# ZhengyiLuo/PULSE

Hardware: AMD Instinct MI355X
Metric: env-steps/sec through PPO update (higher is better)
Workload: dtype f32; 1 GPU; cfg2: 4096 SMPL-humanoid envs/GPU x horizon 32, imitation obs/reward/reset + PPO (actor+critic MLP [1024, 512], minibatch 16384 x 6 mini-epochs); num_envs_per_gpu=4096, horizon=32, global_batch=131072, parallelism=dp1, reference_motion=HBM-resident motion library (1024 clips), queried every step

## Files before the change

### include/pulse_hip.h

```cpp
#ifndef PULSE_HIP_H
#define PULSE_HIP_H

#include <stddef.h>
#include <stdint.h>

#ifdef __cplusplus
extern "C" {
#endif

#define PULSE_OK 0
#define PULSE_ERR_INVALID_ARG (-1)
#define PULSE_ERR_LAUNCH (-2)
#define PULSE_ERR_UNSUPPORTED (-3)

#define PULSE_ABI_VERSION 34

typedef void* pulse_stream_t;

int pulse_abi_version(void);
const char* pulse_last_error(void);

int pulse_quat_mul(const float* a, const float* b, float* out, int64_t m, pulse_stream_t s);
int pulse_quat_conjugate(const float* a, float* out, int64_t m, pulse_stream_t s);
int pulse_quat_rotate(const float* q, const float* v, float* out, int64_t m, pulse_stream_t s);
int pulse_quat_to_angle_axis(const float* q, float* angle, float* axis, int64_t m, pulse_stream_t s);
int pulse_quat_to_exp_map(const float* q, float* out, int64_t m, pulse_stream_t s);
int pulse_quat_to_tan_norm(const float* q, float* out, int64_t m, pulse_stream_t s);
int pulse_exp_map_to_quat(const float* e, float* out, int64_t m, pulse_stream_t s);
int pulse_slerp(const float* q0, const float* q1, const float* t, float* out, int64_t m, pulse_stream_t s);
int pulse_calc_heading(const float* q, float* out, int64_t m, pulse_stream_t s);
int pulse_calc_heading_quat(const float* q, float* out, int64_t m, int inverse, pulse_stream_t s);

typedef struct pulse_motion_tables {
    const float* frames;
    int64_t frame_stride;
    int64_t total_frames;
    int32_t num_bodies;
    int32_t off_gts, off_grs, off_lrs, off_gvs, off_gavs, off_dvs;
    const float* motion_lengths;
    const float* motion_dt;
    const int64_t* motion_num_frames;
    const int64_t* length_starts;
    int32_t num_motions;
} pulse_motion_tables;

typedef struct pulse_reward_specs {
    float k_pos, k_rot, k_vel, k_ang_vel;
    float w_pos, w_rot, w_vel, w_ang_vel;
    float power_coef;
    int32_t power_reward;
} pulse_reward_specs;

#define PULSE_IM_SELF_OBS 1u
#define PULSE_IM_TASK_OBS 2u
#define PULSE_IM_REWARD   4u
#define PULSE_IM_RESET    8u
#define PULSE_IM_DEBUG_POISON_LDS 0x80000000u
#define PULSE_IM_FORCE_WIDE 0x40000000u

typedef struct pulse_im_step_args {
    const float* rb;
    int64_t rb_env_stride;
    int32_t num_envs;
    int32_t num_bodies;
    const int64_t* env_ids;
    int32_t num_ids;
    const uint8_t* env_mask;

// ... 178 lines not shown
    const int64_t* clip_out_start;
    const int64_t* clip_frames_host;
    const float* clip_dt;
    const float* clip_heading;
    const float* local_translation;
    const int32_t* parent_indices_host;
    float* frames;
    int64_t total_frames;
    int64_t frame_stride;
    int32_t off_gts, off_grs, off_lrs, off_gvs, off_gavs, off_dvs;
    float filter_w[9];
} pulse_motion_build_args;
int pulse_sizeof_motion_build_args(void);
int pulse_motion_build(const pulse_motion_build_args* args, pulse_stream_t s);

typedef struct pulse_im_eval_args {
    const float* rb;
    int64_t rb_env_stride;
    const float* ref_pos;
    int64_t ref_env_stride;
    int32_t num_envs;
    int32_t num_bodies;
    const int32_t* num_steps;
    int32_t step;
    const uint8_t* env_mask;
    float* ring;
    double* accum;
    int64_t accum_stride;
} pulse_im_eval_args;
int pulse_sizeof_im_eval_args(void);
int pulse_im_eval_accum(const pulse_im_eval_args* args, pulse_stream_t s);

typedef struct pulse_rollout_record_args {
    int32_t num_envs;
    const float* rewards;
    float reward_scale, reward_shift;
    const int64_t* dones;
    const int64_t* terminate;
    const float* value_raw; int64_t value_stride;
    const double* value_mean; const double* value_var;
    float value_eps;
    float* buf_rewards; float* buf_next_values; uint8_t* buf_dones; int64_t env_stride;
    float* current_rewards; float* current_lengths;
    float* meter_rewards; float* meter_lengths;
    float meter_max_size;
    uint8_t* done_mask;
    uint8_t* buf_terminate;
    float* meter_partials; int32_t meter_blocks;
} pulse_rollout_record_args;
int pulse_sizeof_rollout_record_args(void);
int pulse_rollout_record(const pulse_rollout_record_args* args, pulse_stream_t s);
int pulse_rollout_meters(const float* partials, int32_t steps, int32_t blocks, float* meter_rewards, float* meter_lengths, float meter_max_size,
                         pulse_stream_t s);

int pulse_kinematic_sim_step(const float* target_rb, const float* noise_rb, float* rb, int64_t num_envs, int32_t num_bodies,
                             const float* target_dof_pos, const float* noise_dof_pos, float* dof_pos,
                             const float* target_dof_vel, const float* noise_dof_vel, float* dof_vel,
                             const float* force_src, float* dof_force, int32_t num_dof, pulse_stream_t s);

typedef struct pulse_pd_sim_args {
    int64_t num_envs; int32_t num_bodies;
    const float* target_rb;
    const float* target_dof_pos; const float* target_dof_vel;
    const float* action;
    const float* noise_acc;
    const float* sag;
    const float* lever_dir;
    float kp, kd, dt, action_scale, lever; int32_t substeps;
    float* err; float* err_vel;
    float* rb; float* dof_pos; float* dof_vel; float* dof_force;
    const uint8_t* reset_mask;
} pulse_pd_sim_args;
int pulse_sizeof_pd_sim_args(void);
int pulse_pd_sim_step(const pulse_pd_sim_args* args, pulse_stream_t s);

typedef struct pulse_traj_step_args {
    uint32_t what; int32_t num_envs;
    const int64_t* env_ids; int32_t num_ids; const uint8_t* env_mask;
    const float* rb; int64_t rb_env_stride; int32_t num_bodies;
    int32_t upright_start;
    const int64_t* progress; float dt;
    const float* verts; int32_t num_verts; float traj_dur;
    int32_t num_samples; float sample_timestep;
    const int16_t* heightsamples; int32_t map_rows, map_cols; float horizontal_scale, vertical_scale;
    const float* height_points; int32_t num_height_points; int32_t sensor_body;
    const float* center_points; int32_t num_center_points; int32_t use_center_height; float height_meas_scale;
    const float* dof_force; const float* dof_vel; int32_t num_dof; float power_coef; int32_t power_reward; int32_t fuzzy_target;
    const float* contact_forces; const int32_t* contact_body_ids; int32_t num_contact_ids; const float* termination_heights;
    float max_episode_length, fail_dist; int32_t enable_early_termination, terrain_reset, disable_collision;
    float* obs; int64_t obs_stride; int32_t obs_offset;
    float* rew; float* rew_raw;
    int64_t* reset; int64_t* terminate;
} pulse_traj_step_args;
int pulse_sizeof_traj_step_args(void);
int pulse_traj_step(const pulse_traj_step_args* args, pulse_stream_t s);

typedef struct pulse_traj_gen_args {
    int32_t num_envs, num_verts; const uint8_t* env_mask;
    const float* rb; int64_t rb_env_stride;
    const float* u_dtheta; const float* u_sharp; const uint8_t* sharp_mask; const float* u_heading; const float* u_dspeed; const float* u_speed0;
    float dtheta_scale, dspeed_scale, seg_dt, speed_min, speed_max;
    float* verts;
} pulse_traj_gen_args;
int pulse_traj_generate(const pulse_traj_gen_args* args, pulse_stream_t s);

int pulse_gae(const float* rewards, const float* values, const float* next_values, const uint8_t* dones,
// ... 216 lines not shown
```

### pulse_amd/_lib.py

```python
import ctypes
import os
from ctypes import POINTER, Structure, c_char_p, c_float, c_int, c_int32, c_int64, c_uint32, c_void_p

_HERE = os.path.dirname(os.path.abspath(__file__))
LIB_PATH = os.environ.get("PULSE_HIP_LIB") or os.path.join(_HERE, "csrc", "libpulse_hip.so")
ABI_VERSION = 34

PULSE_IM_SELF_OBS = 1
PULSE_IM_TASK_OBS = 2
PULSE_IM_REWARD = 4
PULSE_IM_RESET = 8
PULSE_IM_DEBUG_POISON_LDS = 0x80000000
PULSE_IM_FORCE_WIDE = 0x40000000


class PulseLibraryError(RuntimeError):
    pass


class RewardSpecs(Structure):
    _fields_ = [("k_pos", c_float), ("k_rot", c_float), ("k_vel", c_float), ("k_ang_vel", c_float),
                ("w_pos", c_float), ("w_rot", c_float), ("w_vel", c_float), ("w_ang_vel", c_float),
                ("power_coef", c_float), ("power_reward", c_int32)]


class MotionTables(Structure):
    _fields_ = [("frames", c_void_p), ("frame_stride", c_int64), ("total_frames", c_int64), ("num_bodies", c_int32),
                ("off_gts", c_int32), ("off_grs", c_int32), ("off_lrs", c_int32), ("off_gvs", c_int32), ("off_gavs", c_int32),
                ("off_dvs", c_int32),
                ("motion_lengths", c_void_p), ("motion_dt", c_void_p), ("motion_num_frames", c_void_p), ("length_starts", c_void_p),
                ("num_motions", c_int32)]


class MotionBuildArgs(Structure):
    _fields_ = [("src_rot", c_void_p), ("src_trans", c_void_p), ("src_frames", c_int64), ("num_clips", c_int32), ("num_bodies", c_int32),
                ("clip_src_start", c_void_p), ("clip_crop_start", c_void_p), ("clip_out_start", c_void_p), ("clip_frames_host", c_void_p),
                ("clip_dt", c_void_p), ("clip_heading", c_void_p), ("local_translation", c_void_p), ("parent_indices_host", c_void_p),
                ("frames", c_void_p), ("total_frames", c_int64), ("frame_stride", c_int64),
                ("off_gts", c_int32), ("off_grs", c_int32), ("off_lrs", c_int32), ("off_gvs", c_int32), ("off_gavs", c_int32), ("off_dvs", c_int32),
                ("filter_w", c_float * 9)]


class ImEvalArgs(Structure):
    _fields_ = [("rb", c_void_p), ("rb_env_stride", c_int64), ("ref_pos", c_void_p), ("ref_env_stride", c_int64), ("num_envs", c_int32),
                ("num_bodies", c_int32), ("num_steps", c_void_p), ("step", c_int32), ("env_mask", c_void_p), ("ring", c_void_p),
                ("accum", c_void_p), ("accum_stride", c_int64)]


class ImStepArgs(Structure):
    _fields_ = [
        ("rb", c_void_p), ("rb_env_stride", c_int64), ("num_envs", c_int32), ("num_bodies", c_int32),
        ("env_ids", c_void_p), ("num_ids", c_int32), ("env_mask", c_void_p),
        ("ref_now_pos", c_void_p), ("ref_now_rot", c_void_p), ("ref_now_vel", c_void_p), ("ref_now_ang", c_void_p),
        ("ref_next_pos", c_void_p), ("ref_next_rot", c_void_p), ("ref_next_vel", c_void_p), ("ref_next_ang", c_void_p),
        ("time_steps", c_int32),
        ("dof_force", c_void_p), ("dof_vel", c_void_p), ("num_dof", c_int32),
        ("progress", c_void_p), ("pass_time", c_void_p), ("cycle_counter", c_void_p),
        ("track_ids", c_void_p), ("num_track", c_int32), ("reset_ids", c_void_p), ("num_reset", c_int32),
        ("term_dist", c_void_p), ("reset_use_mean", c_int32), ("full_body_reward", c_int32),
# ... 178 lines not shown
        ("mu", c_void_p), ("mu_stride", c_int64), ("value", c_void_p), ("value_stride", c_int64), ("logstd", c_void_p),
        ("idx", c_void_p), ("actions", c_void_p), ("actions_stride", c_int64), ("old_mu", c_void_p), ("old_mu_stride", c_int64),
        ("old_logstd", c_void_p), ("old_neglogp", c_void_p), ("advantages", c_void_p), ("old_values", c_void_p), ("returns", c_void_p),
        ("rows", c_int32), ("num_actions", c_int32),
        ("e_clip", c_float), ("critic_coef", c_float), ("bounds_loss_coef", c_float), ("clip_value", c_int32), ("has_bounds_loss", c_int32),
        ("dmu", c_void_p), ("dmu_stride", c_int64), ("dvalue", c_void_p), ("dvalue_stride", c_int64),
        ("partials", c_void_p), ("num_blocks", c_int32),
        ("dmu16", c_void_p), ("dmu16_stride", c_int64), ("dvalue16", c_void_p), ("dvalue16_stride", c_int64),
    ]


GEMM_RED_CONTIG, GEMM_OUT_CONTIG = 0, 1
GEMM_COMPUTE_F32, GEMM_COMPUTE_BF16, GEMM_COMPUTE_F32X3 = 0, 1, 2
ACT_NONE, ACT_RELU, ACT_SILU, ACT_SILU_D = 0, 1, 2, 3
EPI_BIAS_ACT, EPI_RELU_GRAD, EPI_SILU_GRAD, EPI_MUL_AUX = 0, 1, 2, 3

P = c_void_p
c_double = ctypes.c_double

SIGNATURES = {
    "pulse_abi_version": (c_int, []),
    "pulse_last_error": (c_char_p, []),
    "pulse_quat_mul": (c_int, [P, P, P, c_int64, P]),
    "pulse_quat_conjugate": (c_int, [P, P, c_int64, P]),
    "pulse_quat_rotate": (c_int, [P, P, P, c_int64, P]),
    "pulse_quat_to_angle_axis": (c_int, [P, P, P, c_int64, P]),
    "pulse_quat_to_exp_map": (c_int, [P, P, c_int64, P]),
    "pulse_quat_to_tan_norm": (c_int, [P, P, c_int64, P]),
    "pulse_exp_map_to_quat": (c_int, [P, P, c_int64, P]),
    "pulse_slerp": (c_int, [P, P, P, P, c_int64, P]),
    "pulse_calc_heading": (c_int, [P, P, c_int64, P]),
    "pulse_calc_heading_quat": (c_int, [P, P, c_int64, c_int, P]),
    "pulse_sizeof_im_step_args": (c_int, []),
    "pulse_self_obs_width": (c_int, [c_int, c_int]),
    "pulse_task_obs_width": (c_int, [c_int, c_int, c_int]),
    "pulse_self_obs_width_ex": (c_int, [c_int, c_int, c_int, c_int, c_int]),
    "pulse_im_step": (c_int, [POINTER(ImStepArgs), P]),
    "pulse_sizeof_task_step_args": (c_int, []),
    "pulse_task_obs_size": (c_int, [c_int]),
    "pulse_task_step": (c_int, [POINTER(TaskStepArgs), P]),
    "pulse_gemm_set_option": (c_int, [c_int, c_int]),
    "pulse_gemm_set_debug_buffer": (c_int, [P]),
    "pulse_gemm_last_tile": (c_int, []),
    "pulse_gemm_x3_mode": (c_int, []),
    "pulse_sizeof_amp_obs_args": (c_int, []),
    "pulse_amp_obs_width": (c_int, [c_int, c_int, c_int]),
    "pulse_amp_obs_width_v": (c_int, [c_int, c_int, c_int, c_int, c_int, c_int]),
    "pulse_amp_obs": (c_int, [POINTER(AmpObsArgs), P]),
    "pulse_sizeof_amp_hist_args": (c_int, []),
    "pulse_amp_hist_init": (c_int, [POINTER(AmpHistArgs), P]),
    "pulse_sizeof_rollout_record_args": (c_int, []),
    "pulse_rollout_record": (c_int, [POINTER(RolloutRecordArgs), P]),
    "pulse_rollout_meters": (c_int, [P, c_int32, c_int32, P, P, c_float, P]),
    "pulse_kinematic_sim_step": (c_int, [P, P, P, c_int64, c_int32, P, P, P, P, P, P, P, P, c_int32, P]),
    "pulse_sizeof_pd_sim_args": (c_int, []),
    "pulse_pd_sim_step": (c_int, [POINTER(PdSimArgs), P]),
    "pulse_sizeof_motion_state_args": (c_int, []),
    "pulse_motion_state": (c_int, [POINTER(MotionStateArgs), P]),
    "pulse_sizeof_motion_build_args": (c_int, []),
    "pulse_motion_build": (c_int, [POINTER(MotionBuildArgs), P]),
    "pulse_sizeof_im_eval_args": (c_int, []),
    "pulse_im_eval_accum": (c_int, [POINTER(ImEvalArgs), P]),
    "pulse_gae": (c_int, [P, P, P, P, c_int32, c_int32, c_int64, c_int64, c_float, c_float, P, P, P]),
    "pulse_sizeof_gemm_desc": (c_int, []),
    "pulse_gemm_f32": (c_int, [POINTER(GemmDesc), P]),
    "pulse_gemm_x3p": (c_int, [POINTER(GemmX3pDesc), P]),
    "pulse_gemm_x3p_row_tiles": (c_int, [c_int32, c_int32, c_int32]),
    "pulse_traj_step": (c_int, [POINTER(TrajStepArgs), P]),
    "pulse_sizeof_traj_step_args": (c_int, []),
    "pulse_traj_generate": (c_int, [POINTER(TrajGenArgs), P]),
    "pulse_vae_embed": (c_int, [POINTER(VaeEmbedArgs), P]),
    "pulse_vae_kin_loss": (c_int, [POINTER(VaeKinArgs), P]),
    "pulse_vae_head_backward": (c_int, [POINTER(VaeHeadBwdArgs), P]),
    "pulse_sizeof_vae_embed_args": (c_int, []),
    "pulse_sizeof_vae_kin_args": (c_int, []),
    "pulse_sizeof_vae_head_bwd_args": (c_int, []),
    "pulse_mcp_compose": (c_int, [P, c_int64, P, c_int64, c_int32, c_int32, c_int32, c_int32, c_int32, P, c_int64, P]),
    "pulse_mcp_head_forward": (c_int, [P, c_int64, c_int32, c_int32, P, c_int64, P]),
    "pulse_mcp_head_backward": (c_int, [P, c_int64, P, c_int64, P, c_int64, c_int32, c_int32, c_int32, P, c_int64, P]),
    "pulse_sizeof_gemm_x3p_desc": (c_int, []),
    "pulse_split_planes": (c_int, [P, c_int64, c_int32, c_int32, P, c_int64, c_int32, c_int32, P, P]),
    "pulse_reduce_slabs": (c_int, [P, c_int32, c_int64, c_int64, P, c_float, P]),
    "pulse_colsum_partial": (c_int, [P, c_int32, c_int32, c_int32, c_int32, P, c_int64, P]),
    "pulse_rms_normalize": (c_int, [P, c_int64, P, c_int32, c_int32, P, P, c_float, c_float, c_int32, P, c_int64, c_int32, P, c_int32, P]),
    "pulse_rms_normalize_copy": (c_int, [P, c_int64, P, c_int32, c_int32, P, P, c_float, c_float, P, c_int64, c_int32, P, c_int32, P, c_int64, P]),
    "pulse_rms_normalize_planes": (c_int, [P, c_int64, P, c_int32, c_int32, P, P, c_float, c_float, P, c_int64, c_int32, P, c_int32, P, c_int64, c_int64, P]),
    "pulse_rms_normalize_b16": (c_int, [P, c_int64, P, c_int32, c_int32, P, P, c_float, c_float, P, c_int64, c_int32, P, c_int32, P]),
    "pulse_transpose_to_b16": (c_int, [P, c_int64, c_int32, c_int32, P, c_int64, c_int32, c_int64, c_int64, P]),
    "pulse_colsum_partial_b16": (c_int, [P, c_int32, c_int32, c_int64, c_int32, P, c_int64, P]),
    "pulse_colsum_weighted_b16": (c_int, [P, c_int32, c_int32, c_int64, P, c_int64, c_int32, P, c_int64, P]),
    "pulse_disc_penalty": (c_int, [P, c_int64, c_int32, c_int32, c_float, P, c_int64, P, c_int64, P, c_int32, P]),
    "pulse_disc_reg": (c_int, [P, P, c_int32, POINTER(c_int64), POINTER(c_int64), POINTER(c_float), P, c_int32, P]),
    "pulse_sizeof_b16_transpose": (c_int, []),
    "pulse_weights_to_b16": (c_int, [P, c_int64, P, c_int32, POINTER(B16Transpose), P]),
    "pulse_reduce_grads": (c_int, [P, c_int64, c_int32, POINTER(c_int64), POINTER(c_int64), POINTER(c_int32), POINTER(c_float), POINTER(ctypes.c_void_p),
                                   POINTER(c_int64), P, c_float, P, P, P, c_int32, P]),
    "pulse_disc_reward": (c_int, [P, c_int64, c_int64, c_float, P, c_int64, P]),
    "pulse_disc_head_b16": (c_int, [P, c_int64, c_int32, c_float, P, c_int64, P, c_int64, P, P, P]),
    "pulse_rms_update": (c_int, [P, P, P, P, c_int32, c_int32, c_double, c_double, P]),
    "pulse_policy_sample": (c_int, [P, c_int64, P, P, c_int64, P, c_int64, P, P, c_int32, c_int32, P, c_int64, P, c_int64, P, c_int64, P, c_int64, P, c_int64, P]),
    "pulse_sizeof_ppo_loss_args": (c_int, []),
    "pulse_ppo_loss": (c_int, [POINTER(PpoLossArgs), P]),
    "pulse_advantage_moments": (c_int, [P, P, c_int64, P, P, c_int32, P]),
    "pulse_advantage_normalize": (c_int, [P, c_int64, P, c_int32, P]),
    "pulse_sqnorm_partial": (c_int, [P, c_int64, P, c_int32, P]),
    "pulse_disc_head": (c_int, [P, c_int64, c_int32, c_float, P, c_int64, P, P]),
# ... 41 lines not shown
```

### pulse_amd/csrc/rollout_ops.hip

```cpp
#include "common.h"
#include "rot_math.h"

namespace pulse {

__device__ __forceinline__ float wave_sum_f(float v) {
#pragma unroll
    for (int o = 32; o > 0; o >>= 1) v += __shfl_xor(v, o, 64);
    return v;
}

__device__ __forceinline__ void meter_update(float* st, float sum, float count, float max_size) {
    if (count <= 0.f) return;
    const float new_mean = sum / count;
    const float size = fminf(fmaxf(count, 0.f), max_size);
    const float old_size = fminf(max_size - size, st[1]);
    const float size_sum = old_size + size;
    st[0] = (st[0] * old_size + new_mean * size) / size_sum;
    st[1] = size_sum;
}

__global__ void __launch_bounds__(1024) rollout_record_kernel(const pulse_rollout_record_args a) {
    __shared__ float red[3][16];
    float cnt = 0.f, sr = 0.f, sl = 0.f;
    float vs = 1.f, vm = 0.f;
    if (a.value_mean) {
        vs = sqrtf((float)a.value_var[0] + a.value_eps);
        vm = (float)a.value_mean[0];
    }
    const int per = (a.num_envs + gridDim.x - 1) / gridDim.x;
    const int e0 = blockIdx.x * per, e1 = min(a.num_envs, e0 + per);
    for (int e = e0 + threadIdx.x; e < e1; e += blockDim.x) {
        const float r = a.rewards[e];
        const bool done = a.dones[e] != 0;
        const long long o = (long long)e * a.env_stride;
        a.buf_rewards[o] = (a.reward_scale == 1.f && a.reward_shift == 0.f) ? r : (r + a.reward_shift) * a.reward_scale;
        a.buf_dones[o] = done ? 1 : 0;
        if (a.buf_terminate) a.buf_terminate[o] = a.terminate[e] != 0 ? 1 : 0;
        if (a.buf_next_values) {
            float v = a.value_raw[(long long)e * a.value_stride];
            if (a.value_mean) v = vs * fminf(fmaxf(v, -5.f), 5.f) + vm;
            a.buf_next_values[o] = v * (1.0f - (float)a.terminate[e]);
        }
        const float cr = a.current_rewards[e] + r;
        const float cl = a.current_lengths[e] + 1.f;
        if (done) { cnt += 1.f; sr += cr; sl += cl; }
        const float keep = 1.0f - (done ? 1.f : 0.f);
        a.current_rewards[e] = cr * keep;
        a.current_lengths[e] = cl * keep;
        a.done_mask[e] = done ? 1 : 0;
    }
    cnt = wave_sum_f(cnt); sr = wave_sum_f(sr); sl = wave_sum_f(sl);
    const int w = threadIdx.x >> 6;
    if ((threadIdx.x & 63) == 0) { red[0][w] = cnt; red[1][w] = sr; red[2][w] = sl; }
    __syncthreads();
    if (threadIdx.x == 0) {
        float c = 0.f, r = 0.f, l = 0.f;
        const int nw = blockDim.x >> 6;
        for (int i = 0; i < nw; ++i) { c += red[0][i]; r += red[1][i]; l += red[2][i]; }
        if (a.meter_partials) {
            float* o = a.meter_partials + 4 * blockIdx.x;
            o[0] = c; o[1] = r; o[2] = l; o[3] = 0.f;
        } else {
            meter_update(a.meter_rewards, r, c, a.meter_max_size);
            meter_update(a.meter_lengths, l, c, a.meter_max_size);
        }
    }
}

__global__ void rollout_meters_kernel(const float* __restrict__ partials, int steps, int blocks, float* __restrict__ meter_rewards,
                                      float* __restrict__ meter_lengths, float max_size) {
    if (threadIdx.x != 0 || blockIdx.x != 0) return;
    for (int t = 0; t < steps; ++t) {
        float c = 0.f, r = 0.f, l = 0.f;
        for (int b = 0; b < blocks; ++b) {
            const float* p = partials + ((long long)t * blocks + b) * 4;
            c += p[0]; r += p[1]; l += p[2];
        }
        meter_update(meter_rewards, r, c, max_size);
        meter_update(meter_lengths, l, c, max_size);
    }
}

__global__ void __launch_bounds__(256) kinematic_sim_kernel(const float* __restrict__ trb, const float* __restrict__ nrb, float* __restrict__ rb,
                                                           long long bodies, const float* __restrict__ tdp, const float* __restrict__ ndp,
                                                           float* __restrict__ dp, const float* __restrict__ tdv, const float* __restrict__ ndv,
                                                           float* __restrict__ dv, const float* __restrict__ fsrc, float* __restrict__ f, long long dofs) {
    const long long i = (long long)blockIdx.x * 256 + threadIdx.x;
    if (i < bodies) {
        const float* t = trb + i * 13;
        const float* n = nrb + i * 13;
        float v[13];
#pragma unroll
        for (int k = 0; k < 13; ++k) v[k] = t[k] + n[k];
        const float nq = sqrtf(v[3] * v[3] + v[4] * v[4] + v[5] * v[5] + v[6] * v[6]);
#pragma unroll
        for (int k = 3; k < 7; ++k) v[k] = v[k] / nq;
        float* o = rb + i * 13;
#pragma unroll
        for (int k = 0; k < 13; ++k) o[k] = v[k];
    }
    if (i < dofs) {
        dp[i] = tdp[i] + ndp[i];
        dv[i] = tdv[i] + ndv[i];
        f[i] = fsrc[i];
    }
}

__global__ void __launch_bounds__(256) pd_sim_kernel(const pulse_pd_sim_args a) {
    const long long i = (long long)blockIdx.x * 256 + threadIdx.x;
    const int J = a.num_bodies, nd = 3 * (J - 1);
    if (i >= a.num_envs * J) return;
    const long long e = i / J;
    const int b = (int)(i - e * J);
    const float* t = a.target_rb + i * 13;
    float* o = a.rb + i * 13;
    if (b == 0) {
#pragma unroll
        for (int k = 0; k < 13; ++k) o[k] = t[k];
        return;
    }
    const long long d0 = e * nd + 3 * (b - 1);
    const bool rst = a.reset_mask && a.reset_mask[e];
    float er[3], ev[3], tq[3];
    const float h = a.dt / (float)a.substeps;
#pragma unroll
    for (int k = 0; k < 3; ++k) {
        er[k] = rst ? 0.0f : a.err[d0 + k];
        ev[k] = rst ? 0.0f : a.err_vel[d0 + k];
        tq[k] = 0.0f;
    }
    if (!rst) {
        for (int s = 0; s < a.substeps; ++s) {
#pragma unroll
// ... 23 lines not shown
    const V3 cv{ev[1] * u[2] - ev[2] * u[1], ev[2] * u[0] - ev[0] * u[2], ev[0] * u[1] - ev[1] * u[0]};
    const Q4 q = qmul(exp_map_to_q(V3{er[0], er[1], er[2]}), Q4{t[3], t[4], t[5], t[6]});
    o[0] = t[0] + a.lever * ce.x; o[1] = t[1] + a.lever * ce.y; o[2] = t[2] + a.lever * ce.z;
    o[3] = q.x; o[4] = q.y; o[5] = q.z; o[6] = q.w;
    o[7] = t[7] + a.lever * cv.x; o[8] = t[8] + a.lever * cv.y; o[9] = t[9] + a.lever * cv.z;
    o[10] = t[10] + ev[0]; o[11] = t[11] + ev[1]; o[12] = t[12] + ev[2];
}

}

using namespace pulse;

extern "C" int pulse_sizeof_pd_sim_args(void) { return (int)sizeof(pulse_pd_sim_args); }

extern "C" int pulse_pd_sim_step(const pulse_pd_sim_args* args, pulse_stream_t s) {
    PULSE_REQUIRE(args != nullptr, "pulse_pd_sim_step: null args");
    const pulse_pd_sim_args& a = *args;
    PULSE_REQUIRE(a.num_envs >= 0 && a.num_bodies >= 2 && a.substeps >= 1 && a.dt > 0.f, "pulse_pd_sim_step: bad sizes");
    if (a.num_envs == 0) return PULSE_OK;
    PULSE_REQUIRE(a.target_rb && a.target_dof_pos && a.target_dof_vel && a.action && a.noise_acc && a.sag && a.lever_dir && a.err && a.err_vel &&
                      a.rb && a.dof_pos && a.dof_vel && a.dof_force, "pulse_pd_sim_step: null pointer");
    const long long n = a.num_envs * a.num_bodies;
    hipLaunchKernelGGL(pd_sim_kernel, dim3((unsigned)((n + 255) / 256)), dim3(256), 0, as_stream(s), a);
    return check_launch("pulse_pd_sim_step");
}

extern "C" int pulse_sizeof_rollout_record_args(void) { return (int)sizeof(pulse_rollout_record_args); }

extern "C" int pulse_rollout_record(const pulse_rollout_record_args* args, pulse_stream_t s) {
    PULSE_REQUIRE(args != nullptr, "pulse_rollout_record: null args");
    const pulse_rollout_record_args& a = *args;
    PULSE_REQUIRE(a.num_envs >= 0, "pulse_rollout_record: negative num_envs");
    if (a.num_envs == 0) return PULSE_OK;
    PULSE_REQUIRE(a.rewards && a.dones && a.buf_rewards && a.buf_dones && a.current_rewards && a.current_lengths && a.meter_rewards &&
                      a.meter_lengths && a.done_mask, "pulse_rollout_record: null pointer");
    PULSE_REQUIRE(a.buf_next_values == nullptr || (a.value_raw && a.terminate), "pulse_rollout_record: next_values needs value_raw and terminate");
    PULSE_REQUIRE(a.buf_terminate == nullptr || a.terminate, "pulse_rollout_record: buf_terminate needs terminate");
    PULSE_REQUIRE((a.value_mean == nullptr) == (a.value_var == nullptr), "pulse_rollout_record: value_mean / value_var go together");
    PULSE_REQUIRE(a.env_stride >= 1 && a.meter_max_size >= 1.f, "pulse_rollout_record: bad env_stride / meter_max_size");
    if (a.meter_partials) {
        PULSE_REQUIRE(a.meter_blocks >= 1 && a.meter_blocks <= 1024, "pulse_rollout_record: meter_blocks must be in [1, 1024]");
        hipLaunchKernelGGL(rollout_record_kernel, dim3((unsigned)a.meter_blocks), dim3(256), 0, as_stream(s), a);
    } else {
        hipLaunchKernelGGL(rollout_record_kernel, dim3(1), dim3(1024), 0, as_stream(s), a);
    }
    return check_launch("pulse_rollout_record");
}

extern "C" int pulse_rollout_meters(const float* partials, int32_t steps, int32_t blocks, float* meter_rewards, float* meter_lengths, float meter_max_size,
                                    pulse_stream_t s) {
    PULSE_REQUIRE(steps >= 0 && blocks >= 1, "pulse_rollout_meters: bad sizes");
    if (steps == 0) return PULSE_OK;
    PULSE_REQUIRE(partials && meter_rewards && meter_lengths && meter_max_size >= 1.f, "pulse_rollout_meters: bad arguments");
    hipLaunchKernelGGL(rollout_meters_kernel, dim3(1), dim3(64), 0, as_stream(s), partials, steps, blocks, meter_rewards, meter_lengths, meter_max_size);
    return check_launch("pulse_rollout_meters");
}

extern "C" int pulse_kinematic_sim_step(const float* target_rb, const float* noise_rb, float* rb, int64_t num_envs, int32_t num_bodies,
                                        const float* target_dof_pos, const float* noise_dof_pos, float* dof_pos,
                                        const float* target_dof_vel, const float* noise_dof_vel, float* dof_vel,
                                        const float* force_src, float* dof_force, int32_t num_dof, pulse_stream_t s) {
    PULSE_REQUIRE(num_envs >= 0 && num_bodies >= 1 && num_dof >= 1, "pulse_kinematic_sim_step: bad sizes");
    if (num_envs == 0) return PULSE_OK;
    PULSE_REQUIRE(target_rb && noise_rb && rb && target_dof_pos && noise_dof_pos && dof_pos && target_dof_vel && noise_dof_vel && dof_vel &&
                      force_src && dof_force, "pulse_kinematic_sim_step: null pointer");
    const long long bodies = (long long)num_envs * num_bodies, dofs = (long long)num_envs * num_dof;
    const long long n = bodies > dofs ? bodies : dofs;
    hipLaunchKernelGGL(kinematic_sim_kernel, dim3((unsigned)((n + 255) / 256)), dim3(256), 0, as_stream(s), target_rb, noise_rb, rb, bodies,
                       target_dof_pos, noise_dof_pos, dof_pos, target_dof_vel, noise_dof_vel, dof_vel, force_src, dof_force, dofs);
    return check_launch("pulse_kinematic_sim_step");
}
```

### pulse_amd/env/humanoid_im.py

```python
import contextlib
import os

import torch

from .. import ops
from .. import synthetic as syn
from . import env_keys
from .._lib import PULSE_IM_RESET, PULSE_IM_REWARD, PULSE_IM_SELF_OBS, PULSE_IM_TASK_OBS


class Box:

    def __init__(self, low, high, shape):
        import numpy as np
        self.shape = tuple(shape)
        self.low = np.full(self.shape, low, dtype=np.float32)
        self.high = np.full(self.shape, high, dtype=np.float32)


def _env_dict(cfg):
    env = cfg.get("env", cfg)
    if "env" in env and isinstance(env["env"], dict):
        env = env["env"]
    return env


def check_humanoid_options(cfg, task="HumanoidIm"):
    robot = cfg.get("robot", None) if isinstance(cfg, dict) else None
    robot = robot if isinstance(robot, dict) else {}
    ht = robot.get("humanoid_type", "smpl")
    syn.skeleton(ht)
    if ht == "smpl":
        return ht
    env = _env_dict(cfg)
    opt = lambda k, d=False: env.get(k, robot.get(k, d))
    not_built = lambda what, why: NotImplementedError(f"humanoid_type {ht!r} with {what}: not built -- {why}")
    if task != "HumanoidIm":
        raise not_built(task, "the get-up task (humanoid_im_getup.py) and the downstream tasks of env/humanoid_tasks.py (humanoid_speed.py, "
                              "humanoid_reach.py, humanoid_strike.py, humanoid_pedestrian_terrain.py) are built for the 24-body SMPL humanoid")
    if opt("enable_amp_obs"):
        raise not_built("enable_amp_obs", "the AMP frame kernel maps lane = body inside 32 lanes and the 10-step window of the 52-body frame "
                                          "(4 840 columns, humanoid_amp.py:91-118, 925-969) exceeds amp_obs.hip's kAmpMaxW and the normaliser's 3072 columns")
    if opt("occl_training"):
        raise not_built("occl_training", "the reference's mask update indexes columns 9 .. 23 (humanoid_im.py:1046-1058) and the step kernel "
                                         "packs the mask into one 32-bit word per env")
    for k in ("has_shape_obs", "has_weight_obs"):
        if opt(k):
            raise not_built(k, "the shape / limb-weight rows (humanoid.py:266-268, 657-661, 739-878) are filled from SMPL assets")
    if opt("distill") or opt("save_kin_info"):
        raise not_built("distill / save_kin_info", "the distillation teacher (humanoid_im_distill.py:44-63, 143-231) is a 24-body PHC policy")
    if env.get("z_type") is not None or "embedding_size" in env:
        raise not_built("z_type / embedding_size (the amp_z network)", "PULSE-X uses 48 latents (env_pulsex_amp.yaml; amp_network_z_builder.py:32) and vae_head.hip holds "
                                                                       "embedding_size <= 32")
    return ht


def eval_body_names(body_names, humanoid_type="smpl"):
# ... 323 lines not shown
        if self._use_motion_lib and self._amp_fused:
            ops.amp_hist_init(self._motion_lib, self._sampled_motion_ids, self._motion_start_times, self.dt, mask, self._amp_obs_buf, self._key_body_ids,
                              joint_ids=self._amp_joint_ids, local_root_obs=self._local_root_obs, root_height_obs=self._amp_root_height_obs,
                              shape_params=self._amp_motion_shape_rows, limb_weights=self._amp_motion_limb_rows, **self._amp_variant)
            return
        if self._use_motion_lib:
            steps = -self.dt * (torch.arange(0, s, device=self.device) + 1)
            times = (self._motion_start_times.unsqueeze(-1) + steps).view(-1)
            n = self.num_envs
            bufs = self._ref_bufs.setdefault("hist", {})
            ids = self._sampled_motion_ids.repeat_interleave(s)
            res = self._motion_lib.query(ids, times, out=bufs, fields=("rb_records", "dof_pos", "dof_vel"))
            hist = ops.build_amp_observations_smpl(res["rb_records"], res["dof_pos"], res["dof_vel"], self._key_body_ids, joint_ids=self._amp_joint_ids, zero_joints=(),
                                                   local_root_obs=self._local_root_obs, root_height_obs=self._amp_root_height_obs,
                                                   **self._amp_motion_rows(ids), **self._amp_variant)
            hist = hist.view(n, s, self._num_amp_obs_per_step)
        else:
            hist = self._curr_amp_obs_buf.unsqueeze(1).expand(-1, s, -1)
        self._hist_amp_obs_buf.copy_(torch.where(mask[:, None, None], hist, self._hist_amp_obs_buf))

    def _amp_motion_rows(self, motion_ids):
        return {"shape_params": self._amp_motion_shape_rows[motion_ids] if self._amp_motion_shape_rows is not None else None,
                "limb_weights": self._amp_motion_limb_rows[motion_ids] if self._amp_motion_limb_rows is not None else None}

    def fetch_amp_obs_demo(self, num_samples):
        s = self._num_amp_obs_steps
        if self._use_motion_lib:
            lib = self._motion_lib
            ids = lib.sample_motions(num_samples, generator=self._clock_gen)
            t0 = lib.sample_time_interval(ids, generator=self._clock_gen)
            steps = -self.dt * torch.arange(0, s, device=self.device)
            times = (t0.unsqueeze(-1) + steps).view(-1)
            bufs = self._ref_bufs["demo"] if self._ref_bufs["demo"].get("dof_pos", torch.empty(0)).shape[0] == num_samples * s else {}
            res = lib.query(ids.repeat_interleave(s), times, out=bufs, with_records=True)
            self._ref_bufs["demo"] = res
            rb, dp, dv = res["rb_records"], res["dof_pos"], res["dof_vel"]
            rows = self._amp_motion_rows(ids.repeat_interleave(s))
        else:
            rb, dp, dv = self._motion_lib.sample_demo_states(num_samples * s)
            body = (torch.arange(num_samples, device=self.device) % self.num_envs).repeat_interleave(s)
            rows = {"shape_params": self._amp_shape_rows[body] if self._amp_shape_rows is not None else None,
                    "limb_weights": self._amp_limb_rows[body] if self._amp_limb_rows is not None else None}
        out = ops.build_amp_observations_smpl(rb, dp, dv, self._key_body_ids, joint_ids=self._amp_joint_ids, zero_joints=(), local_root_obs=self._local_root_obs,
                                              root_height_obs=self._amp_root_height_obs, **rows, **self._amp_variant)
        out = out.view(num_samples, s * self._num_amp_obs_per_step)
        if self._add_amp_input_noise:
            self._last_amp_noise = torch.randn(out.shape, device=self.device, generator=self._clock_gen if self._use_motion_lib else None)
            out = out + self._last_amp_noise * 0.01
        return out

    def get_task_obs_size_detail(self):
        return self._task_obs_size_detail

    def step(self, actions):
        if self.save_kin_info:
            self.kin_dict["gt_action"] = self._teacher.forward(self._obs_store) if self._teacher is not None else self.sim.gt_action
            self.kin_dict["progress_buf"] = self.progress_buf.clone()
            self.extras["kin_dict"] = self.kin_dict
        self.pre_physics_step(actions)
        self._physics_step()
        self.post_physics_step()

    def _action_to_pd_targets(self, action):
        if self._res_action:
            pd_tar = self._track["dof_pos"] + self._pd_action_scale * action
            pd_lower = self.sim.dof_pos - torch.pi / 2
            pd_upper = self.sim.dof_pos + torch.pi / 2
            return torch.maximum(torch.minimum(pd_tar, pd_upper), pd_lower)
        return torch.addcmul(self._pd_action_offset, self._pd_action_scale, action)

    def pre_physics_step(self, actions):
        self.actions = actions
        if (self.cycle_motion or (self.zero_out_far and self.zero_out_far_train)) and self._use_motion_lib:
            self._update_cycle_count()
        if self._occl_training:
            self._update_occl_training()
        self.sim.set_dof_position_target_tensor(self._action_to_pd_targets(actions))

    def _physics_step(self):
        self.sim.simulate_and_refresh()

    def _update_pass_time(self):
        if self.cycle_motion:
            torch.ge(self.progress_buf, self.max_episode_length - 1, out=self._pass_time)
        else:
            t = self.progress_buf * self.dt + self._motion_start_times + self._motion_start_times_offset
            torch.ge(t, self._motion_len_env, out=self._pass_time)

    def _im_step(self, what, env_ids=None, env_mask=None, ref_next=None, inc=0, obs_copy=None):
        need_now = what & (PULSE_IM_REWARD | PULSE_IM_RESET)
        if self._use_motion_lib:
            clock, motion = self._motion_kwargs(inc)
            ref_now = ref_next = None
        else:
            clock = motion = None
            ref_now = self._ref_now() if need_now else None
            ref_next = (ref_next if ref_next is not None else self._ref_next()) if what & PULSE_IM_TASK_OBS else None
        rb = self.sim.rigid_body_state
        extra = {}
        if self.self_obs_v == 2:
            self._rb_hist[:, -1] = rb
            rb = self._rb_hist
        elif self.self_obs_v == 3:
            extra["force_sensor"] = self._force_sensor
        if self.obs_v == 2:
            extra["dof_pos"] = self.sim.dof_pos
        if self._has_shape_obs:
            extra["smpl_params"] = self.humanoid_shapes[:, :-6]
        if self._has_limb_weight_obs:
            extra["limb_weights"] = self.humanoid_limb_and_weights
        rc = self._recovery_counter_for_step()
        if rc is not None:
            extra["recovery_counter"] = rc
        if self.zero_out_far:
            extra["zero_out_far"] = {"point_goal": self._point_goal, "close_distance": self.close_distance, "far_distance": self.far_distance}
        if self._occl_training:
            extra["occl_bits"], extra["occl_reset"] = self._occl_bits, not (self.zero_out_far and self.zero_out_far_train)
        cache = self._im_launch_cache.setdefault((what, inc, env_ids is None, env_mask is None), {})
        return ops.im_step(
            rb, cache=cache, what=what, ref_now=ref_now, ref_next=ref_next, upright=self._has_upright_start,
            enable_early_termination=self._enable_early_termination, self_obs_version=self.self_obs_v, **extra,
            time_steps=self._num_traj_samples, dof_force=self.sim.dof_force, dof_vel=self.sim.dof_vel,
            progress=self.progress_buf, pass_time=self._pass_time, cycle_counter=self._cycle_counter,
            track_ids=self._track_bodies_id, reset_ids=self._reset_bodies_id, term_dist=self._termination_distances,
            reset_use_mean=self.im_eval and not self.strict_eval, full_body_reward=self._full_body_reward, obs_version=self.obs_v,
            local_root_obs=self._local_root_obs, root_height_obs=self._root_height_obs, specs=self.reward_specs,
            power_coef=self.power_coefficient, power_reward=self.power_reward, env_ids=env_ids, env_mask=env_mask,
            obs=self._obs_store, obs_cols=self.obs_pitch, rew=self.rew_buf, rew_raw=self.reward_raw,
            reset=self.reset_buf, terminate=self._terminate_buf, clock=clock, motion=motion, obs_copy=obs_copy)

# ... 247 lines not shown
        if self._use_motion_lib:
            random_start = self._state_init_random and not self.test
            if random_start:
                self._reset_phase.uniform_(0.0, 1.0, generator=self._clock_gen)
            sim = self.sim
            self._motion_lib.query(self._sampled_motion_ids, offset=self._global_offset, dt=self.dt, start_offsets=self._motion_start_times_offset,
                                   out={"rb_records": sim.rigid_body_state, "dof_pos": sim.dof_pos, "dof_vel": sim.dof_vel},
                                   fields=("rb_records", "dof_pos", "dof_vel"),
                                   reset={"mask": mask, "phase": self._reset_phase if random_start else None, "time_interval": True,
                                          "start_times": self._motion_start_times, "progress": self.progress_buf,
                                          "clear0": self.reset_buf, "clear1": self._terminate_buf, "clear2": self._cycle_counter,
                                          "zero_start_offsets": self._motion_start_times_offset, "zero_global_offset": self._global_offset})
            if hasattr(sim, "on_reset"):
                sim.on_reset(mask)
            if self.zero_out_far and self.zero_out_far_train:
                xy = self._far_start_xy()
                self._global_offset[:, 0:2] = torch.where(mask[:, None], xy, self._global_offset[:, 0:2])
                self._cycle_counter.masked_fill_(mask, self._zero_out_far_steps)
            if self.self_obs_v == 2:
                self._init_tensor_history(mask)
            self._compute_observations(env_mask=mask)
            if self._enable_amp_obs:
                self._init_amp_obs(mask)
            return
        keep = ~mask
        self.sim.set_env_states_masked(mask)
        self.progress_buf.mul_(keep)
        ref_next = self._motion_lib.next_after_reset()
        self.reset_buf.mul_(keep)
        self._terminate_buf.mul_(keep)
        if self.self_obs_v == 2:
            self._init_tensor_history(mask)
        self._compute_observations(env_mask=mask, ref_next=ref_next)
        if self._enable_amp_obs:
            self._init_amp_obs(mask)


class VecTaskPythonWrapper:

    def __init__(self, task, rl_device="cuda:0", clip_observations=float("inf"), clip_actions=1.0):
        self.task = task
        self.env = self
        self.num_envs = task.num_envs
        self.num_obs = task.num_obs
        self.num_actions = task.num_actions
        self.clip_obs, self.clip_actions = clip_observations, clip_actions
        self.obs_space = Box(-float("inf"), float("inf"), (self.num_obs,))
        self.act_space = Box(-1.0, 1.0, (self.num_actions,))
        self.rl_device = rl_device
        self.alias_obs = False
        self.obs_carries_over = True

    def step(self, actions):
        actions_tensor = torch.clamp(actions, -self.clip_actions, self.clip_actions)
        self.task.step(actions_tensor)
        obs = self.task.obs_buf
        if self.clip_obs != float("inf"):
            obs = torch.clamp(obs, -self.clip_obs, self.clip_obs)
        elif not self.alias_obs:
            obs = obs.clone()
        return obs, self.task.rew_buf, self.task.reset_buf, self.task.extras

    def set_obs_sink(self, rows):
        f = getattr(self.task, "set_obs_sink", None)
        if f is None or self.clip_obs != float("inf") or not self.alias_obs:
            return False
        return bool(f(rows))

    def obs_sink_written(self):
        return bool(getattr(self.task, "obs_sink_written", False))

    def reset(self, env_ids=None):
        self.task.reset(env_ids)
        return self.task.obs_buf

    def reset_masked(self, mask):
        self.task.reset_masked(mask)
        return self.task.obs_buf

    def get_number_of_agents(self):
        return 1

    def get_env_info(self):
        info = {"action_space": self.act_space, "observation_space": self.obs_space, "task_obs_size": self.task.get_task_obs_size()}
        if getattr(self.task, "_enable_amp_obs", False):
            info["amp_observation_space"] = self.task._amp_obs_space
            info["enc_amp_observation_space"] = self.task._amp_obs_space
        return info

    def fetch_amp_obs_demo(self, num_samples):
        return self.task.fetch_amp_obs_demo(num_samples)
```

### pulse_amd/kernels.py

```python
import ctypes
import os

import torch

from . import _lib
from ._lib import ACT_NONE, ACT_RELU, ACT_SILU, EPI_BIAS_ACT, GEMM_RED_CONTIG, GemmDesc, PpoLossArgs
from .ops import _dev, _ptr, _stream

ACTIVATIONS = {"None": ACT_NONE, "none": ACT_NONE, None: ACT_NONE, "relu": ACT_RELU, "silu": ACT_SILU}


def _p(t):
    return t.data_ptr() if t is not None else None


def _chk(t, name, dtype=torch.float32, contiguous=True):
    if t is None:
        return None
    if not isinstance(t, torch.Tensor) or t.device.type != "cuda":
        raise TypeError(f"{name}: expected a CUDA tensor, got {type(t).__name__} on {getattr(t, 'device', None)}")
    if t.dtype != dtype and not (dtype == torch.uint8 and t.dtype == torch.bool):
        raise TypeError(f"{name}: expected dtype {dtype}, got {t.dtype}")
    if contiguous and t.numel() > 0 and t.stride(-1) != 1:
        raise ValueError(f"{name}: innermost stride must be 1, got strides {tuple(t.stride())}")
# ... 725 lines not shown


def adam_step_multi(groups, *, lr, step, beta1=0.9, beta2=0.999, eps=1e-8, weight_decay=0.0, max_norm=0.0, sqnorm_partials=None, grad_norm_out=None):
    n = len(groups)
    if not 1 <= n <= 4:
        raise ValueError("adam_step_multi: 1..4 groups")
    _chk(sqnorm_partials, "sqnorm_partials"), _chk(grad_norm_out, "grad_norm_out")
    cols = [[], [], [], []]
    for g in groups:
        for k, nm in enumerate(("params", "grads", "exp_avg", "exp_avg_sq")):
            _chk(g[k], nm)
            if g[k].numel() < g[4] or not g[k].is_contiguous():
                raise ValueError(f"adam_step_multi: {nm} must be a contiguous buffer of at least {g[4]} floats")
            cols[k].append(g[k].data_ptr())
    arrs = [(ctypes.c_void_p * n)(*c) for c in cols]
    counts = (ctypes.c_int64 * n)(*[int(g[4]) for g in groups])
    _lib.check(_lib.load().pulse_adam_step_multi(n, arrs[0], arrs[1], arrs[2], arrs[3], counts, float(lr), beta1, beta2, eps, weight_decay, int(step),
                                                 float(max_norm), _p(sqnorm_partials), sqnorm_partials.numel() if sqnorm_partials is not None else 0,
                                                 _p(grad_norm_out), _stream()), "pulse_adam_step_multi")


def rollout_record(*, rewards, dones, terminate, value_raw, value_stride, value_mean, value_var, value_eps, buf_rewards, buf_next_values,
                   buf_dones, env_stride, current_rewards, current_lengths, meter_rewards, meter_lengths, meter_max_size, done_mask,
                   reward_scale=1.0, reward_shift=0.0, buf_terminate=None, meter_partials=None):
    a = _lib.RolloutRecordArgs()
    a.num_envs = rewards.numel()
    a.rewards, a.reward_scale, a.reward_shift = _chk(rewards, "rewards"), float(reward_scale), float(reward_shift)
    a.dones, a.terminate = _chk(dones, "dones", torch.int64), _chk(terminate, "terminate", torch.int64)
    _chk(done_mask, "done_mask", torch.uint8), _chk(current_rewards, "current_rewards"), _chk(current_lengths, "current_lengths")
    _chk(meter_rewards, "meter_rewards"), _chk(meter_lengths, "meter_lengths"), _chk(value_mean, "value_mean", torch.float64)
    _chk(value_var, "value_var", torch.float64)
    a.value_raw, a.value_stride = _p(value_raw), int(value_stride)
    a.value_mean, a.value_var, a.value_eps = _p(value_mean), _p(value_var), float(value_eps)
    a.buf_rewards, a.buf_next_values, a.buf_dones, a.env_stride = _p(buf_rewards), _p(buf_next_values), _p(buf_dones), int(env_stride)
    a.current_rewards, a.current_lengths = _p(current_rewards), _p(current_lengths)
    a.meter_rewards, a.meter_lengths, a.meter_max_size = _p(meter_rewards), _p(meter_lengths), float(meter_max_size)
    a.done_mask, a.buf_terminate = _p(done_mask), _p(buf_terminate)
    if meter_partials is not None:
        _chk(meter_partials, "meter_partials")
        if meter_partials.dim() != 2 or meter_partials.shape[1] != 4 or not meter_partials.is_contiguous():
            raise ValueError("rollout_record: meter_partials must be a contiguous (blocks, 4) tensor")
        a.meter_partials, a.meter_blocks = meter_partials.data_ptr(), meter_partials.shape[0]
    _lib.check(_lib.load().pulse_rollout_record(ctypes.byref(a), _stream()), "pulse_rollout_record")


def rollout_meters(partials, meter_rewards, meter_lengths, meter_max_size):
    _chk(partials, "partials"), _chk(meter_rewards, "meter_rewards"), _chk(meter_lengths, "meter_lengths")
    if partials.dim() != 3 or partials.shape[2] != 4 or not partials.is_contiguous():
        raise ValueError("rollout_meters: partials must be a contiguous (steps, blocks, 4) tensor")
    _lib.check(_lib.load().pulse_rollout_meters(partials.data_ptr(), partials.shape[0], partials.shape[1], meter_rewards.data_ptr(), meter_lengths.data_ptr(),
                                               float(meter_max_size), _stream()), "pulse_rollout_meters")


def kinematic_sim_step(target_rb, noise_rb, rb, target_dof_pos, noise_dof_pos, dof_pos, target_dof_vel, noise_dof_vel, dof_vel, force_src,
                       dof_force):
    n, j = rb.shape[0], rb.shape[1]
    _lib.check(_lib.load().pulse_kinematic_sim_step(_p(target_rb), _p(noise_rb), _p(rb), n, j, _p(target_dof_pos), _p(noise_dof_pos),
                                                    _p(dof_pos), _p(target_dof_vel), _p(noise_dof_vel), _p(dof_vel), _p(force_src),
                                                    _p(dof_force), dof_pos.shape[1], _stream()), "pulse_kinematic_sim_step")
```

Measured before the change: 1.934 million env-steps/s.

## Fuse action clamp with PD target and parallelize rollout meter reduction

Adds a pd_target kernel that clamps actions and computes the PD targets (offset + scale*clamped) in one launch, replacing the separate torch.clamp and addcmul. The env wrapper now passes the clip value down to HumanoidIm, which uses the fused kernel when its shape and stride conditions hold. Separately, the rollout meters kernel gives each of up to 256 threads one step's partial sums, read as float4 loads, instead of one thread looping over every step and block. The meter updates themselves still run serially on thread 0, so their order is unchanged.

```diff
diff --git a/include/pulse_hip.h b/include/pulse_hip.h
--- a/include/pulse_hip.h
+++ b/include/pulse_hip.h
@@ -13,7 +13,7 @@
 #define PULSE_ERR_LAUNCH (-2)
 #define PULSE_ERR_UNSUPPORTED (-3)
 
-#define PULSE_ABI_VERSION 34
+#define PULSE_ABI_VERSION 35
 
 typedef void* pulse_stream_t;
 
@@ -298,6 +298,9 @@
 int pulse_rollout_record(const pulse_rollout_record_args* args, pulse_stream_t s);
 int pulse_rollout_meters(const float* partials, int32_t steps, int32_t blocks, float* meter_rewards, float* meter_lengths, float meter_max_size,
                          pulse_stream_t s);
+
+int pulse_pd_target(const float* actions, int64_t actions_stride, float clip, const float* offset, const float* scale, float* out, float* clamped,
+                    int64_t rows, int32_t cols, pulse_stream_t s);
 
 int pulse_kinematic_sim_step(const float* target_rb, const float* noise_rb, float* rb, int64_t num_envs, int32_t num_bodies,
                              const float* target_dof_pos, const float* noise_dof_pos, float* dof_pos,
diff --git a/pulse_amd/_lib.py b/pulse_amd/_lib.py
--- a/pulse_amd/_lib.py
+++ b/pulse_amd/_lib.py
@@ -4,7 +4,7 @@
 
 _HERE = os.path.dirname(os.path.abspath(__file__))
 LIB_PATH = os.environ.get("PULSE_HIP_LIB") or os.path.join(_HERE, "csrc", "libpulse_hip.so")
-ABI_VERSION = 34
+ABI_VERSION = 35
 
 PULSE_IM_SELF_OBS = 1
 PULSE_IM_TASK_OBS = 2
@@ -289,6 +289,7 @@
     "pulse_sizeof_rollout_record_args": (c_int, []),
     "pulse_rollout_record": (c_int, [POINTER(RolloutRecordArgs), P]),
     "pulse_rollout_meters": (c_int, [P, c_int32, c_int32, P, P, c_float, P]),
+    "pulse_pd_target": (c_int, [P, c_int64, c_float, P, P, P, P, c_int64, c_int32, P]),
     "pulse_kinematic_sim_step": (c_int, [P, P, P, c_int64, c_int32, P, P, P, P, P, P, P, P, c_int32, P]),
     "pulse_sizeof_pd_sim_args": (c_int, []),
     "pulse_pd_sim_step": (c_int, [POINTER(PdSimArgs), P]),
diff --git a/pulse_amd/csrc/rollout_ops.hip b/pulse_amd/csrc/rollout_ops.hip
--- a/pulse_amd/csrc/rollout_ops.hip
+++ b/pulse_amd/csrc/rollout_ops.hip
@@ -67,18 +67,50 @@
     }
 }
 
-__global__ void rollout_meters_kernel(const float* __restrict__ partials, int steps, int blocks, float* __restrict__ meter_rewards,
-                                      float* __restrict__ meter_lengths, float max_size) {
-    if (threadIdx.x != 0 || blockIdx.x != 0) return;
-    for (int t = 0; t < steps; ++t) {
-        float c = 0.f, r = 0.f, l = 0.f;
-        for (int b = 0; b < blocks; ++b) {
-            const float* p = partials + ((long long)t * blocks + b) * 4;
-            c += p[0]; r += p[1]; l += p[2];
-        }
-        meter_update(meter_rewards, r, c, max_size);
-        meter_update(meter_lengths, l, c, max_size);
-    }
+constexpr int kMeterSteps = 256;
+__global__ void __launch_bounds__(kMeterSteps) rollout_meters_kernel(const float* __restrict__ partials, int steps, int blocks,
+                                                                     float* __restrict__ meter_rewards, float* __restrict__ meter_lengths, float max_size) {
+    __shared__ float sums[3][kMeterSteps];
+    for (int t0 = 0; t0 < steps; t0 += kMeterSteps) {
+        const int t = t0 + (int)threadIdx.x;
+        if (t < steps) {
+            const float4* p = reinterpret_cast<const float4*>(partials) + (long long)t * blocks;
+            float c = 0.f, r = 0.f, l = 0.f;
+            int b = 0;
+            for (; b + 8 <= blocks; b += 8) {
+                float4 v[8];
+#pragma unroll
+                for (int u = 0; u < 8; ++u) v[u] = p[b + u];
+#pragma unroll
+                for (int u = 0; u < 8; ++u) { c += v[u].x; r += v[u].y; l += v[u].z; }
+            }
+            for (; b < blocks; ++b) { const float4 v = p[b]; c += v.x; r += v.y; l += v.z; }
+            sums[0][threadIdx.x] = c; sums[1][threadIdx.x] = r; sums[2][threadIdx.x] = l;
+        }
+        __syncthreads();
+        if (threadIdx.x == 0) {
+            const int n = min(kMeterSteps, steps - t0);
+            for (int i = 0; i < n; ++i) {
+                meter_update(meter_rewards, sums[1][i], sums[0][i], max_size);
+                meter_update(meter_lengths, sums[2][i], sums[0][i], max_size);
+            }
+        }
+        __syncthreads();
+    }
+}
+
+__global__ void __launch_bounds__(256) pd_target_kernel(const float* __restrict__ actions, long long actions_stride, float clip,
+                                                       const float* __restrict__ offset, const float* __restrict__ scale, float* __restrict__ out,
+                                                       float* __restrict__ clamped, long long count, int cols) {
+    const long long i = (long long)blockIdx.x * 256 + threadIdx.x;
+    if (i >= count) return;
+    const long long row = i / cols;
+    const int j = (int)(i - row * cols);
+    const float a = actions[row * actions_stride + j];
+    const float c = a != a ? a : fminf(fmaxf(a, -clip), clip);
+    if (clamped) clamped[i] = c;
+    const float prod = scale[j] * c;
+    out[i] = offset[j] + prod;
 }
 
 __global__ void __launch_bounds__(256) kinematic_sim_kernel(const float* __restrict__ trb, const float* __restrict__ nrb, float* __restrict__ rb,
@@ -208,8 +240,20 @@
     PULSE_REQUIRE(steps >= 0 && blocks >= 1, "pulse_rollout_meters: bad sizes");
     if (steps == 0) return PULSE_OK;
     PULSE_REQUIRE(partials && meter_rewards && meter_lengths && meter_max_size >= 1.f, "pulse_rollout_meters: bad arguments");
-    hipLaunchKernelGGL(rollout_meters_kernel, dim3(1), dim3(64), 0, as_stream(s), partials, steps, blocks, meter_rewards, meter_lengths, meter_max_size);
+    PULSE_REQUIRE((reinterpret_cast<uintptr_t>(partials) & 15) == 0, "pulse_rollout_meters: partials must be 16-byte aligned");
+    hipLaunchKernelGGL(rollout_meters_kernel, dim3(1), dim3(kMeterSteps), 0, as_stream(s), partials, steps, blocks, meter_rewards, meter_lengths, meter_max_size);
     return check_launch("pulse_rollout_meters");
+}
+
+extern "C" int pulse_pd_target(const float* actions, int64_t actions_stride, float clip, const float* offset, const float* scale, float* out,
+                               float* clamped, int64_t rows, int32_t cols, pulse_stream_t s) {
+    PULSE_REQUIRE(rows >= 0 && cols >= 1 && actions_stride >= cols, "pulse_pd_target: bad sizes");
+    if (rows == 0) return PULSE_OK;
+    PULSE_REQUIRE(actions && offset && scale && out, "pulse_pd_target: null pointer");
+    PULSE_REQUIRE(rows * cols < (1LL << 31) * 256, "pulse_pd_target: too many elements for one launch");
+    const long long n = (long long)rows * cols;
+    hipLaunchKernelGGL(pd_target_kernel, dim3((unsigned)((n + 255) / 256)), dim3(256), 0, as_stream(s), actions, (long long)actions_stride, clip, offset, scale, out, clamped, n, (int)cols);
+    return check_launch("pulse_pd_target");
 }
 
 extern "C" int pulse_kinematic_sim_step(const float* target_rb, const float* noise_rb, float* rb, int64_t num_envs, int32_t num_bodies,
diff --git a/pulse_amd/env/humanoid_im.py b/pulse_amd/env/humanoid_im.py
--- a/pulse_amd/env/humanoid_im.py
+++ b/pulse_amd/env/humanoid_im.py
@@ -3,6 +3,7 @@
 
 import torch
 
+from .. import kernels as K
 from .. import ops
 from .. import synthetic as syn
 from . import env_keys
@@ -432,12 +433,15 @@
     def get_task_obs_size_detail(self):
         return self._task_obs_size_detail
 
-    def step(self, actions):
+    def step(self, actions, clip=None):
         if self.save_kin_info:
             self.kin_dict["gt_action"] = self._teacher.forward(self._obs_store) if self._teacher is not None else self.sim.gt_action
             self.kin_dict["progress_buf"] = self.progress_buf.clone()
             self.extras["kin_dict"] = self.kin_dict
-        self.pre_physics_step(actions)
+        if clip is None:
+            self.pre_physics_step(actions)
+        else:
+            self.pre_physics_step(actions, clip=clip)
         self._physics_step()
         self.post_physics_step()
 
@@ -449,13 +453,20 @@
             return torch.maximum(torch.minimum(pd_tar, pd_upper), pd_lower)
         return torch.addcmul(self._pd_action_offset, self._pd_action_scale, action)
 
-    def pre_physics_step(self, actions):
+    def pre_physics_step(self, actions, clip=None):
+        pd_tar = None
+        if clip is not None:
+            if (not self._res_action and K.pd_target_supported(actions) and self._pd_action_offset.shape == actions.shape[1:] == self._pd_action_scale.shape
+                    and self._pd_action_offset.is_contiguous() and self._pd_action_scale.is_contiguous()):
+                pd_tar, actions = K.pd_target(actions, clip, self._pd_action_offset, self._pd_action_scale)
+            else:
+                actions = torch.clamp(actions, -clip, clip)
         self.actions = actions
         if (self.cycle_motion or (self.zero_out_far and self.zero_out_far_train)) and self._use_motion_lib:
             self._update_cycle_count()
         if self._occl_training:
             self._update_occl_training()
-        self.sim.set_dof_position_target_tensor(self._action_to_pd_targets(actions))
+        self.sim.set_dof_position_target_tensor(self._action_to_pd_targets(actions) if pd_tar is None else pd_tar)
 
     def _physics_step(self):
         self.sim.simulate_and_refresh()
@@ -809,8 +820,11 @@
         self.obs_carries_over = True
 
     def step(self, actions):
-        actions_tensor = torch.clamp(actions, -self.clip_actions, self.clip_actions)
-        self.task.step(actions_tensor)
+        tt = type(self.task)
+        if tt.step is HumanoidIm.step and tt.pre_physics_step is HumanoidIm.pre_physics_step and tt._action_to_pd_targets is HumanoidIm._action_to_pd_targets:
+            self.task.step(actions, clip=self.clip_actions)
+        else:
+            self.task.step(torch.clamp(actions, -self.clip_actions, self.clip_actions))
         obs = self.task.obs_buf
         if self.clip_obs != float("inf"):
             obs = torch.clamp(obs, -self.clip_obs, self.clip_obs)
diff --git a/pulse_amd/kernels.py b/pulse_amd/kernels.py
--- a/pulse_amd/kernels.py
+++ b/pulse_amd/kernels.py
@@ -801,6 +801,23 @@
                                                float(meter_max_size), _stream()), "pulse_rollout_meters")
 
 
+def pd_target(actions, clip, offset, scale, want_clamped=True):
+    _chk(actions, "actions"), _chk(offset, "offset"), _chk(scale, "scale")
+    if actions.dim() != 2 or offset.shape != actions.shape[1:] or scale.shape != actions.shape[1:] or not pd_target_supported(actions):
+        raise ValueError("pd_target: actions must be (rows, cols) with unit column stride and a row pitch >= cols, offset / scale contiguous (cols,)")
+    rows, cols = actions.shape
+    out = torch.empty(rows, cols, device=actions.device)
+    clamped = torch.empty(rows, cols, device=actions.device) if want_clamped else None
+    _lib.check(_lib.load().pulse_pd_target(_p(actions), actions.stride(0) if rows > 1 else cols, float(clip), _p(offset), _p(scale), _p(out), _p(clamped),
+                                           rows, cols, _stream()), "pulse_pd_target")
+    return out, clamped
+
+
+def pd_target_supported(actions):
+    return (actions.is_cuda and actions.dtype == torch.float32 and actions.dim() == 2 and actions.shape[1] >= 1 and
+            (actions.shape[0] <= 1 or actions.stride(0) >= actions.shape[1]) and (actions.shape[1] == 1 or actions.stride(1) == 1))
+
+
 def kinematic_sim_step(target_rb, noise_rb, rb, target_dof_pos, noise_dof_pos, dof_pos, target_dof_vel, noise_dof_vel, dof_vel, force_src,
                        dof_force):
     n, j = rb.shape[0], rb.shape[1]
```

Result: faster. 1.960 million env-steps/s (median of 6 runs) (+1.4%).
